# xdslproject/ExaHyPE

Hardware: AMD Instinct MI355X
Metric: DoF-updates/sec, 3D Euler p=5 fused STP+volume+Riemann, 1/2/4/8 MI355X (higher is better)
Workload: dtype f64

## Files before the change

### exahype_amd/csrc/exa_dg_reg.hpp

```cpp
#pragma once
#include "exa_dg_kernels.hpp"

namespace exa {

template <class P, class = void> struct pde_has_dir : std::false_type {};
template <class P> struct pde_has_dir<P, std::void_t<typename P::Dir>> : std::true_type {};

template <class PDE, bool HAS = pde_has_dir<PDE>::value> struct DirFlux;
template <class PDE> struct DirFlux<PDE, true> {
    typename PDE::Dir c;
    __device__ inline DirFlux(int d, double sc) { PDE::dir_init(c, d, sc); }
    __device__ inline void operator()(const double* q, const double* a, double* F) const { PDE::flux_scaled_dir(q, a, c, F); }
    __device__ inline double scale() const {
        double a = c.psc[0];
        asm volatile("" : "+v"(a));
        return (a + c.psc[1]) + c.psc[2];
    }
    __device__ inline void put(const double* pv, double vn, double sc, double* F) const { PDE::flux_scaled_put(pv, vn, c, sc, F); }
};
template <class PDE> struct DirFlux<PDE, false> {
    int d;
    double sc;
    __device__ inline DirFlux(int d_, double sc_) : d(d_), sc(sc_) {}
    __device__ inline void operator()(const double* q, const double* a, double* F) const {
        if (d == 0) PDE::template flux_scaled<0>(q, a, sc, F);
        else if (d == 1) PDE::template flux_scaled<1>(q, a, sc, F);
        else PDE::template flux_scaled<2>(q, a, sc, F);
    }
};

template <class P, class = void> struct pde_has_put : std::false_type {};
template <class P> struct pde_has_put<P, std::void_t<decltype(P::NPUT), decltype(P::PUT_VN)>> : std::true_type {};
template <class P, bool HAS = pde_has_put<P>::value> struct pde_nput { static constexpr int value = 0, vn = 0; };
template <class P> struct pde_nput<P, true> { static constexpr int value = P::NPUT, vn = P::PUT_VN; };

#ifndef EXA_REG_CPW
#define EXA_REG_CPW 2
#endif

template <int N> struct RegGeo {
    static constexpr int NN = N * N * N, NF = N * N;
    static constexpr int PY = N, PX = N * N;
    static constexpr int SL = NN + (NN % 2 == 0 ? 1 : 0);
    __host__ __device__ static constexpr int pstride(int d) { return d == 0 ? PX : (d == 1 ? PY : 1); }
    __host__ __device__ static inline int pbase(int d, int t) {
        const int a = t / N, b = t - a * N;
        return d == 0 ? a * PY + b : (d == 1 ? a * PX + b : a * PX + b * PY);
    }
};

template <int N, class PDE, int CPW = 1> struct StageAReg {
    using G = RegGeo<N>;
    static constexpr int NV = PDE::NV, NA = PDE::NAUX;
    static constexpr int NT = 256;
    static constexpr int LG = 2;
    static constexpr int LS = (N + LG - 1) / LG;
    static constexpr int VS = LG * G::SL;
    static constexpr int QSZ = NV * VS;
    static constexpr int NVA = NV + NA;
    static constexpr bool NCPV = pde_has_ncp<PDE>::value;
    static constexpr bool PUT = pde_has_put<PDE>::value && pde_has_dir<PDE>::value && !NCPV && !pde_has_xt<PDE>::value;
    static constexpr int NIMG = PUT ? pde_nput<PDE>::value : NVA;
    static constexpr int SOFF = NIMG * VS;
    static constexpr int GOFF = SOFF;
    static constexpr int PIC_D = SOFF + 3 * QSZ;
    static constexpr int FS = G::NN;
    static constexpr int FIN_D = (pde_has_source<PDE>::value ? 5 : 4) * NV * FS;
    static constexpr int CELL_D = PIC_D > FIN_D ? PIC_D : FIN_D;
    static constexpr size_t LDS_BYTES = sizeof(double) * ((size_t)CELL_D * CPW + 2 * 3 * N);
    static constexpr bool FITS = G::NN <= NT && 2 * sizeof(double) * (size_t)CELL_D + 2048 <= 160 * 1024;
    static constexpr int TAB_INTS = 2 * NT;
};

__device__ inline void lds_barrier() { __syncthreads(); }


template <int N, class PDE, int CPW, bool FUSE = false>
__global__ void __launch_bounds__(256 * CPW, 2)
dg_stage_a_reg_kernel(const double* u_in, double* u_out, double* __restrict__ trace,
                      long ncells, CellBox box, double dt, double idx0, double idx1, double idx2, int n_it,
                      const void* __restrict__ ops_raw, const int* __restrict__ tab, const void* __restrict__ step_raw, RegFuse fz, PlainGeo geo) {
    constexpr bool XT = pde_has_xt<PDE>::value, NCP = pde_has_ncp<PDE>::value;
    constexpr bool FXT = pde_flux_xt<PDE>::value;
    static_assert(!(FUSE && (XT || NCP)), "the one-kernel step is built for term sets without coordinates / ncp");
    using G = RegGeo<N>;
    using SA = StageAReg<N, PDE, CPW>;
    constexpr int NV = SA::NV, NA = SA::NA, DIM = 3;
    constexpr int NN = G::NN, NF = G::NF, SL = G::SL, PX = G::PX, PY = G::PY;
    constexpr int NT = SA::NT, LS = SA::LS, VS = SA::VS, QSZ = SA::QSZ, SOFF = SA::SOFF, FS = SA::FS, NVA = SA::NVA;
    [[maybe_unused]] constexpr int GOFF = SA::GOFF;
    constexpr bool PUT = SA::PUT;
    constexpr int NIMG = SA::NIMG, NLD = PUT ? NIMG + 1 : NVA;
    constexpr int H = N / 2;
    extern __shared__ __attribute__((aligned(16))) double lds_all[];
    const int half = __builtin_amdgcn_readfirstlane(threadIdx.x >> 8);
    const int tid = threadIdx.x & 255;
    __attribute__((address_space(3))) double* lds = (__attribute__((address_space(3))) double*)lds_all + half * SA::CELL_D;
    [[maybe_unused]] const int bt = (tid & 63) + 64 * half, grp = tid >> 6;
    EXA_STAMP_INIT();
    auto bar = [&]() {
        if constexpr (FUSE) {
            __builtin_amdgcn_fence(__ATOMIC_RELEASE, "workgroup", "local");
            __builtin_amdgcn_s_barrier();
            __builtin_amdgcn_fence(__ATOMIC_ACQUIRE, "workgroup", "local");
        } else {
            lds_barrier();
        }
    };
    const bool node_lane = tid < NN;
    const int o_n = node_lane ? tid : 0;
    const int pk2 = tab[tid], pk1 = tab[NT + tid];

    auto ld_group = [&](int base, int idx, auto& out) {
        constexpr int K = sizeof(out) / sizeof(double);
#pragma unroll
        for (int k = 0; k < K; k++) out[k] = EXA_LD(base + k * VS + idx);
    };
    auto st_group = [&](int base, int idx, const auto& in) {
        constexpr int K = sizeof(in) / sizeof(double);
#pragma unroll
        for (int k = 0; k < K; k++) EXA_ST(base + k * VS + idx, in[k]);
    };

    constexpr int NE = H * N + H + 1;
    struct Task {
        int off, ps, so;
        int vo;
        bool on;
        int d, ls;
        double xa, xb;
    };
    auto decode = [&](int pk, Task& k, DirFlux<PDE>& fx) {
        const int d = pk & 3, ls = (pk >> 2) & 1, t = pk >> 3;
        const int a = t / N, b = t - a * N;
        k.on = pk >= 0;
        k.off = ls * SL + (d == 0 ? a * PY + b : (d == 1 ? a * PX + b : a * PX + b * PY));
        k.ps = d == 0 ? PX : (d == 1 ? PY : 1);
        k.so = SOFF + d * QSZ;
        k.vo = PUT ? (pde_nput<PDE>::vn + d) * VS * (int)sizeof(double) : 0;
        k.d = d;
        k.ls = ls;
        if constexpr (XT) {
            k.xa = xi_of<N>(geo, a);
            k.xb = xi_of<N>(geo, b);
        }
        fx = DirFlux<PDE>(d, d == 0 ? idx0 : (d == 1 ? idx1 : idx2));
    };
    [[maybe_unused]] double xc[3] = {0.0, 0.0, 0.0};
    [[maybe_unused]] auto pencil_x = [&](const Task& tk, int d, int jn, double (&x)[3]) {
        const double xj = geo.xi[jn];
        x[0] = xc[0] + (d == 0 ? xj : tk.xa) * geo.h[0];
        x[1] = xc[1] + (d == 1 ? xj : (d == 0 ? tk.xa : tk.xb)) * geo.h[1];
        x[2] = xc[2] + (d == 2 ? xj : tk.xb) * geo.h[2];
    };
    [[maybe_unused]] double xio[3] = {0.0, 0.0, 0.0};
    if constexpr (XT) {
        xio[0] = xi_of<N>(geo, o_n / (N * N));
        xio[1] = xi_of<N>(geo, (o_n / N) % N);
        xio[2] = xi_of<N>(geo, o_n % N);
    }
    [[maybe_unused]] auto owner_x = [&](double (&x)[3]) {
#pragma unroll
        for (int a = 0; a < 3; a++) x[a] = xc[a] + xio[a] * geo.h[a];
    };
    [[maybe_unused]] auto level_t = [&](int l) -> double { return geo.t + geo.xi[l] * dt; };
    [[maybe_unused]] auto source_at = [&](const double* qv, int l, double* S) {
        if constexpr (pde_has_source<PDE>::value) {
            if constexpr (XT) {
                double x[3];
                owner_x(x);
                PDE::source_xt(qv, x, level_t(l), S);
            } else {
                PDE::source(qv, S);
            }
        }
    };
    Task tk2;
    DirFlux<PDE> fx2(0, 0.0);
    decode(pk2, tk2, fx2);
    bool active_now = true;
    static_assert(N % 2 == 0, "register-resident stage A: even N (the middle node of an odd N is not coded)");
    auto derive_a = [&](auto dc, const Task& tk, const DirFlux<PDE>& fx, double (&e)[H][NV], double (&o)[H][NV], [[maybe_unused]] double tA,
                        [[maybe_unused]] double tB) {
        constexpr int DC = decltype(dc)::value;
        if (tk.on && active_now) {
            const int off = tk.off, ps = tk.ps;
            double qa[N][NLD];
            auto ld_node = [&](int jn) {
                if constexpr (PUT) {
                    const volatile __attribute__((address_space(3))) double* a = &lds[off + jn * ps];
#pragma unroll
                    for (int k = 0; k < NIMG; k++) qa[jn][k] = a[k * VS];
                    const volatile __attribute__((address_space(3))) double* b;
                    asm volatile("v_add_u32 %0, %1, %2" : "=v"(b) : "v"(a), "v"(tk.vo));
                    qa[jn][NIMG] = *b;
                } else {
                    ld_group(0, off + jn * ps, qa[jn]);
                }
            };
#pragma unroll
            for (int j = 0; j < H; j++) {
                ld_node(j);
                ld_node(N - 1 - j);
            }
            [[maybe_unused]] double scl = 0.0;
            if constexpr (PUT) scl = fx.scale();
            [[maybe_unused]] const double tl = tk.ls ? tB : tA;
            [[maybe_unused]] const int dd = DC >= 0 ? DC : tk.d;
            [[maybe_unused]] const double scd = dd == 0 ? idx0 : (dd == 1 ? idx1 : idx2);
#pragma unroll
            for (int j = 0; j < H; j++) {
                double Fa[NV], Fb[NV];
                if constexpr (FXT) {
                    double xj[3];
                    pencil_x(tk, dd, j, xj);
                    dg_flux_xt<PDE>(qa[j], xj, tl, dd, Fa);
                    pencil_x(tk, dd, N - 1 - j, xj);
                    dg_flux_xt<PDE>(qa[N - 1 - j], xj, tl, dd, Fb);
#pragma unroll
                    for (int v = 0; v < NV; v++) { Fa[v] *= scd; Fb[v] *= scd; }
                } else if constexpr (DC >= 0) {
                    PDE::template flux_scaled<DC>(qa[j], qa[j] + NV, scd, Fa);
                    PDE::template flux_scaled<DC>(qa[N - 1 - j], qa[N - 1 - j] + NV, scd, Fb);
                } else if constexpr (PUT) {
                    fx.put(qa[j], qa[j][NIMG], scl, Fa);
                    fx.put(qa[N - 1 - j], qa[N - 1 - j][NIMG], scl, Fb);
                } else {
                    fx(qa[j], qa[j] + NV, Fa);
                    fx(qa[N - 1 - j], qa[N - 1 - j] + NV, Fb);
                }
#pragma unroll
                for (int v = 0; v < NV; v++) {
                    e[j][v] = Fa[v] + Fb[v];
                    o[j][v] = Fa[v] - Fb[v];
                }
            }
        }
    };
    [[maybe_unused]] auto derive_g = [&](const Task& tk, [[maybe_unused]] const double (&Em)[NE]) {
        if constexpr (NCP) {
            if (tk.on && active_now) {
                const int off = tk.off, ps = tk.ps, go = GOFF + tk.d * QSZ;
                const double scd = tk.d == 0 ? idx0 : (tk.d == 1 ? idx1 : idx2);
                double e[H][NV], o[H][NV];
#pragma unroll
                for (int j = 0; j < H; j++) {
                    double qa[NV], qb[NV];
                    ld_group(0, off + j * ps, qa);
                    ld_group(0, off + (N - 1 - j) * ps, qb);
#pragma unroll
                    for (int v = 0; v < NV; v++) {
                        e[j][v] = scd * (qa[v] + qb[v]);
                        o[j][v] = scd * (qa[v] - qb[v]);
                    }
                }
#pragma unroll
                for (int i = 0; i < H; i++) {
                    double M[NV], gI[NV], gM[NV];
#pragma unroll
                    for (int v = 0; v < NV; v++) M[v] = Em[H + i] * o[0][v];
#pragma unroll
                    for (int j = 1; j < H; j++)
#pragma unroll
                        for (int v = 0; v < NV; v++) EXA_FMA(M[v], Em[j * N + H + i], o[j][v]);
#pragma unroll
                    for (int v = 0; v < NV; v++) gI[v] = M[v];
#pragma unroll
                    for (int j = 0; j < H; j++)
#pragma unroll
                        for (int v = 0; v < NV; v++) EXA_FMA(gI[v], Em[j * N + i], e[j][v]);
#pragma unroll
                    for (int v = 0; v < NV; v++) gM[v] = fma(2.0, M[v], -gI[v]);
                    st_group(go, off + i * ps, gI);
                    st_group(go, off + (N - 1 - i) * ps, gM);
                }
            }
        }
    };
    [[maybe_unused]] auto ncp_at_owner = [&](const double* qv, int ls, int l, double (&out)[NV]) {
#pragma unroll
        for (int v = 0; v < NV; v++) out[v] = 0.0;
        if constexpr (NCP) {
            double xo[3] = {0.0, 0.0, 0.0};
            if constexpr (XT) owner_x(xo);
            static_for<0, DIM>([&](auto dc) {
                constexpr int D = decltype(dc)::value;
                double g[NV], nd[NV];
                ld_group(GOFF + D * QSZ, o_n + ls * SL, g);
#pragma unroll
                for (int v = 0; v < NV; v++) nd[v] = 0.0;
                dg_ncp<PDE>(qv, g, xo, XT ? level_t(l) : 0.0, D, nd);
#pragma unroll
                for (int v = 0; v < NV; v++) out[v] += nd[v];
            });
        }
    };
    auto derive_b = [&](const Task& tk, const double (&Em)[NE], const double (&e)[H][NV], const double (&o)[H][NV]) {
        if (tk.on && active_now) {
            const int off = tk.off, ps = tk.ps, so = PUT ? opaque_v(tk.so) : tk.so;
#pragma unroll
            for (int i = 0; i < H; i++) {
                double M[NV], sI[NV];
#pragma unroll
                for (int v = 0; v < NV; v++) M[v] = Em[H + i] * o[0][v];
#pragma unroll
                for (int j = 1; j < H; j++)
#pragma unroll
                    for (int v = 0; v < NV; v++) EXA_FMA(M[v], Em[j * N + H + i], o[j][v]);
#pragma unroll
                for (int v = 0; v < NV; v++) sI[v] = M[v];
#pragma unroll
                for (int j = 0; j < H; j++)
#pragma unroll
                    for (int v = 0; v < NV; v++) EXA_FMA(sI[v], Em[j * N + i], e[j][v]);
                double sM[NV];
#pragma unroll
                for (int v = 0; v < NV; v++) sM[v] = fma(2.0, M[v], -sI[v]);
                st_group(so, off + i * ps, sI);
                st_group(so, off + (N - 1 - i) * ps, sM);
            }
        }
    };
    using M0 = std::integral_constant<int, 0>;
    using M1 = std::integral_constant<int, 1>;
    using M2 = std::integral_constant<int, 2>;
    constexpr bool SPLIT_DIR = FXT || !pde_has_dir<PDE>::value;
    auto derive = [&](const Task& tk, const DirFlux<PDE>& fx, const double (&Em)[NE], double tA, double tB, auto mode) {
        __builtin_amdgcn_s_setprio(1);
        double e[H][NV], o[H][NV];
        constexpr int MODE = decltype(mode)::value;
        static_assert(!(NCP && MODE == 0), "gradients and sums share their arrays: two phases (M1, owners, M2)");
        if constexpr (MODE != 2) derive_g(tk, Em);
        auto front = [&](auto dc) {
            if constexpr (MODE != 1) derive_a(dc, tk, fx, e, o, tA, tB);
        };
        if constexpr (SPLIT_DIR) {
            if (tk.d == 0) front(std::integral_constant<int, 0>{});
            else if (tk.d == 1) front(std::integral_constant<int, 1>{});
            else front(std::integral_constant<int, 2>{});
        } else {
            front(std::integral_constant<int, -1>{});
        }
        if constexpr (MODE != 1) {
            derive_b(tk, Em, e, o);
        }
        __builtin_amdgcn_s_setprio(0);
    };

    int cx, cy, cz, sx, sy, sz;
    long trips;
    {
        const long b0 = (long)blockIdx.x * CPW + half, g = (long)gridDim.x * CPW;
        cz = (int)(b0 % box.nb[2]);
        cy = (int)((b0 / box.nb[2]) % box.nb[1]);
        cx = (int)(b0 / (box.nb[2] * box.nb[1]));
        sz = (int)(g % box.nb[2]);
        sy = (int)((g / box.nb[2]) % box.nb[1]);
        sx = (int)(g / (box.nb[2] * box.nb[1]));
        const long first = (long)blockIdx.x * CPW;
        trips = first < box.nbox ? (box.nbox - first + g - 1) / g : 0;
    }
    const int nb0 = (int)box.nb[0], nb1 = (int)box.nb[1], nb2 = (int)box.nb[2];
    auto cell_of = [&](int x, int y, int z) { return ((box.lo[0] + x) * box.nc[1] + box.lo[1] + y) * box.nc[2] + box.lo[2] + z; };
    double un[NV];
#pragma unroll
    for (int v = 0; v < NV; v++) un[v] = (node_lane && cx < nb0) ? u_in[(cell_of(cx, cy, cz) * NN + o_n) * NV + v] : 1.0;
    constexpr int TS = 2 * NV * NF;
    [[maybe_unused]] double tq[FUSE ? 4 : 1][NV];
    [[maybe_unused]] auto face_blocks = [&](int x, int y, int z, const double*& pm, const double*& pp, int& fyl) -> bool {
        const int lt = opaque_v(tid);
        const int f = lt / NF;
        fyl = lt - f * NF;
        const int d = f >> 1, side = f & 1;
        const int c0 = (int)box.lo[0] + x, c1 = (int)box.lo[1] + y, c2 = (int)box.lo[2] + z;
        const int n0 = (int)box.nc[0], n1 = (int)box.nc[1], n2 = (int)box.nc[2];
        const int cell = (c0 * n1 + c1) * n2 + c2;
        const int cst = d == 0 ? n1 * n2 : (d == 1 ? n2 : 1);
        const int ccd = d == 0 ? c0 : (d == 1 ? c1 : c2), ncd = d == 0 ? n0 : (d == 1 ? n1 : n2);
        const int tcell = d == 0 ? c1 * n2 + c2 : (d == 1 ? c0 * n2 + c2 : c0 * n1 + c1);
        const double* gh = f == 0 ? fz.ghost[0] : (f == 1 ? fz.ghost[1] : (f == 2 ? fz.ghost[2] : (f == 3 ? fz.ghost[3] : (f == 4 ? fz.ghost[4] : fz.ghost[5]))));
        const bool inner = side == 0 ? ccd > 0 : ccd < ncd - 1;
        const int nb = inner ? (side == 0 ? cell - cst : cell + cst) : (side == 0 ? cell + (ncd - 1) * cst : cell - (ncd - 1) * cst);
        const double* own = fz.trace_in + ((long)(d * 2 + side) * ncells + cell) * TS;
        const double* oth = (!inner && gh) ? gh + (long)tcell * TS : fz.trace_in + ((long)(d * 2 + 1 - side) * ncells + nb) * TS;
        pm = side == 0 ? oth : own;
        pp = side == 0 ? own : oth;
        return lt < 2 * DIM * NF && x < nb0;
    };
    [[maybe_unused]] auto fetch_faces = [&](int x, int y, int z) {
        if constexpr (FUSE) {
            const double *pm, *pp;
            int fyl;
#ifdef EXA_FUSE_ABL_NOLOAD
            const bool on = face_blocks(x, y, z, pm, pp, fyl) && false;
#else
            const bool on = face_blocks(x, y, z, pm, pp, fyl);
#endif
#pragma unroll
            for (int v = 0; v < NV; v++) {
                tq[0][v] = on ? pm[v * NF + fyl] : 1.0;
                tq[1][v] = on ? pp[v * NF + fyl] : 1.0;
                tq[2][v] = on ? pm[(NV + v) * NF + fyl] : 0.0;
                tq[3][v] = on ? pp[(NV + v) * NF + fyl] : 0.0;
            }
        }
    };
    constexpr int CWT = SA::CELL_D * CPW;
    if constexpr (FUSE) {
        if (threadIdx.x < 2 * DIM * N) {
            const DgOps<N>* og = reinterpret_cast<const DgOps<N>*>(ops_raw);
            const int t = threadIdx.x, D = t / (2 * N), sd = (t / N) & 1, i = t % N;
            const double idd = D == 0 ? idx0 : (D == 1 ? idx1 : idx2);
            ((__attribute__((address_space(3))) double*)lds_all)[CWT + t] = fz.dt_prev * idd * og->iw[i] * (sd == 0 ? og->phiL[i] : og->phiR[i]);
        }
    }
    fetch_faces(cx, cy, cz);
    if constexpr (CPW == 2) {
        if (half == 1) bar();
    }

    constexpr bool DEFER = FUSE;
    [[maybe_unused]] double upend[NV];
    [[maybe_unused]] long pend_cell = -1;
#pragma unroll
    for (int v = 0; v < NV; v++) upend[v] = 0.0;
    for (long trip = 0; trip < trips; trip++) {
        const bool active = cx < nb0;
        active_now = active;
        const bool owner = node_lane && active;
        const long cell = active ? cell_of(cx, cy, cz) : 0;
        if constexpr (XT) {
            xc[0] = geo.x0[0] + (double)(box.lo[0] + cx) * geo.h[0];
            xc[1] = geo.x0[1] + (double)(box.lo[1] + cy) * geo.h[1];
            xc[2] = geo.x0[2] + (double)(box.lo[2] + cz) * geo.h[2];
        }
        cz += sz;
        if (cz >= nb2) { cz -= nb2; cy += 1; }
        cy += sy;
        if (cy >= nb1) { cy -= nb1; cx += 1; }
        cx += sx;

        double q[N][NV];
        double Em[NE];
        sload<NE>(ops_here<N>(ops_raw)->DEO, Em);

        auto put_level = [&](int ls, const double (&qv)[NV]) {
            if constexpr (PUT) {
                double pv[NIMG];
                PDE::put_fast(qv, pv);
                st_group(0, o_n + ls * SL, pv);
            } else {
                double qa[NVA];
#pragma unroll
                for (int v = 0; v < NV; v++) qa[v] = qv[v];
                PDE::aux_fast(qv, qa + NV);
                st_group(0, o_n + ls * SL, qa);
            }
        };
#ifdef EXA_FUSE_ABL_NOPROLOGUE
        if constexpr (FUSE) {
            if (tq[0][0] == 1.2345e-300) un[0] += tq[1][1] + tq[2][2] + tq[3][3];
        }
        if constexpr (false) {
#else
        if constexpr (FUSE) {
#endif
            constexpr int LAM = SOFF, FSO = SOFF + NT;
            const int lt = opaque_v(tid);
            const int ff = lt / NF, fy = lt - ff * NF;
            const bool face_lane = lt < 2 * DIM * NF;
            const int d = ff >> 1;
            const double lam = face_lane ? fmax(PDE::maxeig_fast(tq[0], d), PDE::maxeig_fast(tq[1], d)) : 0.0;
            EXA_ST(LAM + tid, lam);
            bar();
            if (face_lane) {
                double lv[NF];
#pragma unroll
                for (int y = 0; y < NF; y++) lv[y] = EXA_LD(LAM + ff * NF + y);
#pragma unroll
                for (int st = 1; st < NF; st *= 2)
#pragma unroll
                    for (int y = 0; y + st < NF; y += 2 * st) lv[y] = fmax(lv[y], lv[y + st]);
                const double sm = lv[0];
#pragma unroll
                for (int v = 0; v < NV; v++) EXA_ST(FSO + (ff * NV + v) * NF + fy, 0.5 * (tq[2][v] + tq[3][v]) - 0.5 * sm * (tq[1][v] - tq[0][v]));
            }
            bar();
            if (owner) {
                static_for<0, DIM>([&](auto dc) {
                    constexpr int D = decltype(dc)::value;
                    const int on_ = opaque_v(o_n);
                    const int i = (on_ / G::pstride(D)) % N;
                    const int yy = D == 0 ? on_ % (N * N) : (D == 1 ? (on_ / (N * N)) * N + on_ % N : on_ / N);
                    const __attribute__((address_space(3))) double* cwt = (const __attribute__((address_space(3))) double*)lds_all + CWT + D * 2 * N;
                    const double cwL = cwt[i], cwR = cwt[N + i];
#pragma unroll
                    for (int v = 0; v < NV; v++) {
                        const double fL = EXA_LD(FSO + ((2 * D + 0) * NV + v) * NF + yy), fR = EXA_LD(FSO + ((2 * D + 1) * NV + v) * NF + yy);
                        un[v] -= cwR * fR - cwL * fL;
                    }
                });
                if (fz.u_plain) {
#pragma unroll
                    for (int v = 0; v < NV; v++) fz.u_plain[(cell * NN + o_n) * NV + v] = un[v];
                }
            }
        }
        double ukeep[NV];
#pragma unroll
        for (int v = 0; v < NV; v++) ukeep[v] = un[v];
        if constexpr (DEFER) {
            if (node_lane && pend_cell >= 0) {
                double* uo = u_out + (pend_cell * NN + o_n) * NV;
#pragma unroll
                for (int v = 0; v < NV; v++) uo[v] = upend[v];
            }
        }
        if constexpr (XT) {
#pragma unroll
            for (int l = 0; l < N; l++)
#pragma unroll
                for (int v = 0; v < NV; v++) q[l][v] = owner ? un[v] : 1.0;
        } else {
            if (owner) put_level(0, un);
            EXA_STAMP(0);
            bar();
            EXA_STAMP(1);
            [[maybe_unused]] double nd0[NV];
            {
                Task tk1;
                DirFlux<PDE> fx1(0, 0.0);
                decode(opaque_v(pk1), tk1, fx1);
                if constexpr (NCP) {
                    derive(tk1, fx1, Em, 0.0, 0.0, M1{});
                    bar();
                    if (owner) ncp_at_owner(un, 0, 0, nd0);
                    bar();
                    derive(tk1, fx1, Em, 0.0, 0.0, M2{});
                } else {
                    derive(tk1, fx1, Em, 0.0, 0.0, M0{});
                }
            }
            EXA_STAMP(2);
            bar();
            EXA_STAMP(3);
            if (owner) {
                double S[NV], Ts[N];
                sload<N>(step_here<N>(step_raw)->Tsdt, Ts);
                {
                    double Sx[NV], Sy[NV], Sz[NV];
                    ld_group(SOFF, o_n, Sx);
                    ld_group(SOFF + QSZ, o_n, Sy);
                    ld_group(SOFF + 2 * QSZ, o_n, Sz);
    #pragma unroll
                    for (int v = 0; v < NV; v++) S[v] = Sx[v] + (Sy[v] + Sz[v]);
                }
                if constexpr (pde_has_source<PDE>::value) {
                    double Sq[NV];
                    PDE::source(un, Sq);
    #pragma unroll
                    for (int v = 0; v < NV; v++) S[v] -= Sq[v];
                }
                if constexpr (NCP) {
    #pragma unroll
                    for (int v = 0; v < NV; v++) S[v] += nd0[v];
                }
    #pragma unroll
                for (int l = 0; l < N; l++)
    #pragma unroll
                    for (int v = 0; v < NV; v++) q[l][v] = fma(Ts[l], S[v], un[v]);
            } else {
    #pragma unroll
                for (int l = 0; l < N; l++)
    #pragma unroll
                    for (int v = 0; v < NV; v++) q[l][v] = 1.0;
            }
            EXA_STAMP(4);

        }
        auto load_levels = [&](auto lc, const double (&qq)[N][NV]) {
            constexpr int l0 = decltype(lc)::value;
            constexpr int NL = (l0 + 1 < N) ? 2 : 1;
#pragma unroll
            for (int ls = 0; ls < NL; ls++) put_level(ls, qq[l0 + ls]);
        };
        constexpr int IT0 = XT ? 0 : 1;
        if constexpr (PUT) decode(opaque_v(pk2), tk2, fx2);
        if (n_it > IT0 && owner) load_levels(std::integral_constant<int, 0>{}, q);
        constexpr bool DEFER_FOLD = NCP || XT;
        for (int it = IT0; it < n_it; it++) {
            double acc[N][NV];
            [[maybe_unused]] double Sk[DEFER_FOLD ? N : 1][NV];
            static_for<0, LS>([&](auto sc_) {
                constexpr int st = decltype(sc_)::value;
                constexpr int l0 = st * 2;
                constexpr int NL = (l0 + 1 < N) ? 2 : 1;
                sload<NE>(ops_here<N>(ops_raw)->DEO, Em);
                EXA_STAMP(5);
                bar();
                EXA_STAMP(6);
                static_assert(NL == 2, "odd N: the last step of an iteration has one level -- mask the tasks of level slot 1");
                [[maybe_unused]] double ndk[NL][NV];
                if constexpr (NCP) {
                    derive(tk2, fx2, Em, XT ? level_t(l0) : 0.0, XT ? level_t(l0 + 1) : 0.0, M1{});
                    bar();
                    if (owner) {
#pragma unroll
                        for (int ls = 0; ls < NL; ls++) ncp_at_owner(q[l0 + ls], ls, l0 + ls, ndk[ls]);
                    }
                    bar();
                    derive(tk2, fx2, Em, XT ? level_t(l0) : 0.0, XT ? level_t(l0 + 1) : 0.0, M2{});
                } else {
                    derive(tk2, fx2, Em, XT ? level_t(l0) : 0.0, XT ? level_t(l0 + 1) : 0.0, M0{});
                }
                [[maybe_unused]] double Tm[NL * N], uu[NV];
                if constexpr (!DEFER_FOLD) {
#pragma unroll
                    for (int k = 0; k < NL * N; k++) Tm[k] = step_here<N>(step_raw)->TdtT[l0 * N + k];
                    if constexpr (st == 0) {
#pragma unroll
                        for (int v = 0; v < NV; v++) uu[v] = ukeep[v];
                    }
                }
                EXA_STAMP(7);
                bar();
                EXA_STAMP(8);
                if (owner) {
                    if constexpr (!DEFER_FOLD) spin(Tm);
                    double Sx[NL][NV], Sy[NL][NV], Sz[NL][NV];
#pragma unroll
                    for (int ls = 0; ls < NL; ls++) {
                        ld_group(SOFF, o_n + ls * SL, Sx[ls]);
                        ld_group(SOFF + QSZ, o_n + ls * SL, Sy[ls]);
                        ld_group(SOFF + 2 * QSZ, o_n + ls * SL, Sz[ls]);
                    }
                    if constexpr (st + 1 < LS) load_levels(std::integral_constant<int, l0 + 2>{}, q);
                    __builtin_amdgcn_sched_barrier(0);
#pragma unroll
                    for (int ls = 0; ls < NL; ls++)
#pragma unroll
                        for (int v = 0; v < NV; v++) Sx[ls][v] += Sy[ls][v] + Sz[ls][v];
                    if constexpr (pde_has_source<PDE>::value) {
#pragma unroll
                        for (int ls = 0; ls < NL; ls++) {
                            double Sq[NV];
                            source_at(q[l0 + ls], l0 + ls, Sq);
#pragma unroll
                            for (int v = 0; v < NV; v++) Sx[ls][v] -= Sq[v];
                        }
                    }
                    if constexpr (NCP) {
#pragma unroll
                        for (int ls = 0; ls < NL; ls++)
#pragma unroll
                            for (int v = 0; v < NV; v++) Sx[ls][v] += ndk[ls][v];
                    }
                    if constexpr (DEFER_FOLD) {
#pragma unroll
                        for (int ls = 0; ls < NL; ls++)
#pragma unroll
                            for (int v = 0; v < NV; v++) Sk[l0 + ls][v] = Sx[ls][v];
                        if constexpr (st + 1 == LS) {
                            static_for<0, LS>([&](auto s2_) {
                                constexpr int s2 = decltype(s2_)::value;
                                constexpr int m0 = s2 * 2;
                                double T2[NL * N];
                                sload<NL * N>(step_here<N>(step_raw)->TdtT + m0 * N, T2);
#pragma unroll
                                for (int ls = 0; ls < NL; ls++)
#pragma unroll
                                    for (int lp = 0; lp < N; lp++)
#pragma unroll
                                        for (int v = 0; v < NV; v++)
                                            acc[lp][v] = fma(T2[ls * N + lp], Sk[m0 + ls][v], (s2 == 0 && ls == 0) ? ukeep[v] : acc[lp][v]);
                            });
                        }
                    } else {
#pragma unroll
                    for (int ls = 0; ls < NL; ls++)
#pragma unroll
                        for (int lp = 0; lp < N; lp++)
#pragma unroll
                            for (int v = 0; v < NV; v++) {
                                if constexpr (st == 0) acc[lp][v] = fma(Tm[ls * N + lp], Sx[ls][v], ls == 0 ? uu[v] : acc[lp][v]);
                                else acc[lp][v] = fma(Tm[ls * N + lp], Sx[ls][v], acc[lp][v]);
                            }
                    }
                    if constexpr (st + 1 == LS) {
                        if (it + 1 < n_it) load_levels(std::integral_constant<int, 0>{}, acc);
                    }
                }
                EXA_STAMP(9);
            });
#pragma unroll
            for (int l = 0; l < N; l++)
#pragma unroll
                for (int v = 0; v < NV; v++) q[l][v] = owner ? acc[l][v] : 1.0;
        }

        [[maybe_unused]] double pw[NV];
        if constexpr (NCP) {
#pragma unroll
            for (int v = 0; v < NV; v++) pw[v] = 0.0;
            if (owner) load_levels(std::integral_constant<int, 0>{}, q);
            static_for<0, LS>([&](auto sc_) {
                constexpr int st = decltype(sc_)::value;
                constexpr int l0 = st * 2;
                sload<NE>(ops_here<N>(ops_raw)->DEO, Em);
                bar();
                derive(tk2, fx2, Em, XT ? level_t(l0) : 0.0, XT ? level_t(l0 + 1) : 0.0, M1{});
                bar();
                if (owner) {
                    double wl[2];
                    sload<2>(ops_here<N>(ops_raw)->w + l0, wl);
#pragma unroll
                    for (int ls = 0; ls < 2; ls++) {
                        double nd[NV];
                        ncp_at_owner(q[l0 + ls], ls, l0 + ls, nd);
#pragma unroll
                        for (int v = 0; v < NV; v++) pw[v] = fma(wl[ls], nd[v], pw[v]);
                    }
                    if constexpr (st + 1 < LS) load_levels(std::integral_constant<int, l0 + 2>{}, q);
                }
            });
        }
        bar();
        if (owner) {
            double wm[N];
            sload<N>(ops_here<N>(ops_raw)->w, wm);
            double qb[NV], Fb[DIM][NV];
            [[maybe_unused]] double Sbar[NV];
#pragma unroll
            for (int v = 0; v < NV; v++) qb[v] = 0.0;
#pragma unroll
            for (int d = 0; d < DIM; d++)
#pragma unroll
                for (int v = 0; v < NV; v++) Fb[d][v] = 0.0;
            if constexpr (pde_has_source<PDE>::value) {
#pragma unroll
                for (int v = 0; v < NV; v++) Sbar[v] = 0.0;
            }
#pragma unroll
            for (int l = 0; l < N; l++) {
                double a[nz(NA)], F[NV];
                PDE::aux_fast(q[l], a);
#pragma unroll
                for (int v = 0; v < NV; v++) qb[v] += wm[l] * q[l][v];
                static_for<0, DIM>([&](auto dc) {
                    constexpr int D = decltype(dc)::value;
                    if constexpr (FXT) {
                        double xo[3];
                        owner_x(xo);
                        dg_flux_xt<PDE>(q[l], xo, level_t(l), D, F);
                    } else {
                        PDE::template flux<D>(q[l], a, F);
                    }
#pragma unroll
                    for (int v = 0; v < NV; v++) Fb[D][v] += wm[l] * F[v];
                });
                if constexpr (pde_has_source<PDE>::value) {
                    double Sq[NV];
                    source_at(q[l], l, Sq);
#pragma unroll
                    for (int v = 0; v < NV; v++) Sbar[v] += wm[l] * Sq[v];
                }
            }
#pragma unroll
            for (int v = 0; v < NV; v++) {
                EXA_ST(v * FS + o_n, qb[v]);
#pragma unroll
                for (int d = 0; d < DIM; d++) EXA_ST(((1 + d) * NV + v) * FS + o_n, Fb[d][v]);
                if constexpr (pde_has_source<PDE>::value) EXA_ST((4 * NV + v) * FS + o_n, Sbar[v]);
            }
        }
        EXA_STAMP(10);
        bar();

#pragma unroll
        for (int v = 0; v < NV; v++) un[v] = (node_lane && cx < nb0) ? u_in[(cell_of(cx, cy, cz) * NN + o_n) * NV + v] : 1.0;
        fetch_faces(cx, cy, cz);

        {
            double KE[NE], iwm[N], pl[N], pr[N];
            sload<NE>(ops_here<N>(ops_raw)->KEO, KE);
            sload<N>(ops_here<N>(ops_raw)->iw, iwm);
            sload<N>(ops_here<N>(ops_raw)->phiL, pl);
            sload<N>(ops_here<N>(ops_raw)->phiR, pr);
            static_assert(NV * NF <= NT, "closing phases: one round per direction");
            const int tv = PUT ? opaque_v(tid) : tid;
            const int v = tv / NF, t = tv - v * NF;
            static_for<0, DIM>([&](auto dc) {
                constexpr int D = decltype(dc)::value;
                if (tid < NV * NF) {
                    constexpr int ps = G::pstride(D);
                    const int pb = G::pbase(D, t);
                    double qb[N], Fb[N], vol[N];
#pragma unroll
                    for (int j = 0; j < N; j++) {
                        qb[j] = EXA_LD(v * FS + pb + j * ps);
                        Fb[j] = EXA_LD(((1 + D) * NV + v) * FS + pb + j * ps);
                    }
                    eo_apply<N>(KE, Fb, vol);
                    const double sc = dt * (D == 0 ? idx0 : (D == 1 ? idx1 : idx2));
#pragma unroll
                    for (int i = 0; i < N; i++) EXA_ST(((1 + D) * NV + v) * FS + pb + i * ps, sc * iwm[i] * vol[i]);
                    double qL = 0.0, qR = 0.0, FL = 0.0, FR = 0.0;
#pragma unroll
                    for (int j = 0; j < N; j++) {
                        qL += pl[j] * qb[j];
                        qR += pr[j] * qb[j];
                        FL += pl[j] * Fb[j];
                        FR += pr[j] * Fb[j];
                    }
                    if (active) {
                        double* tl = trace + (((long)D * 2 + 0) * ncells + cell) * (2 * NV * NF);
                        double* tr = trace + (((long)D * 2 + 1) * ncells + cell) * (2 * NV * NF);
                        tl[(0 * NV + v) * NF + t] = qL;
                        tl[(1 * NV + v) * NF + t] = FL;
                        tr[(0 * NV + v) * NF + t] = qR;
                        tr[(1 * NV + v) * NF + t] = FR;
                    }
                }
            });
        }
        EXA_STAMP(11);
        bar();

        if (owner) {
            double us[NV];
#pragma unroll
            for (int v2 = 0; v2 < NV; v2++) {
                us[v2] = ukeep[v2];
                if constexpr (NCP) us[v2] -= dt * pw[v2];
                if constexpr (pde_has_source<PDE>::value) us[v2] += dt * EXA_LD((4 * NV + v2) * FS + o_n);
#pragma unroll
                for (int d = 0; d < DIM; d++) us[v2] += EXA_LD(((1 + d) * NV + v2) * FS + o_n);
            }
            if constexpr (DEFER) {
#pragma unroll
                for (int v2 = 0; v2 < NV; v2++) upend[v2] = us[v2];
            } else {
                double* uo = u_out + (cell * NN + o_n) * NV;
#pragma unroll
                for (int v2 = 0; v2 < NV; v2++) uo[v2] = us[v2];
            }
        }
        if constexpr (DEFER) pend_cell = active ? cell : -1;
        bar();
    }
    if constexpr (DEFER) {
        if (node_lane && pend_cell >= 0) {
            double* uo = u_out + (pend_cell * NN + o_n) * NV;
#pragma unroll
            for (int v = 0; v < NV; v++) uo[v] = upend[v];
        }
    }
    if constexpr (CPW == 2) {
        if (half == 0) bar();
    }
    EXA_STAMP_FLUSH();
}

}
```

Baseline: 13.58 billion.

## Relocate closing LDS image past aux area to drop end-of-trip barrier

Moves the closing-phase LDS arrays (q, fluxes, source) to start after the aux image region (offset SOFF) and pads them to the SL stride, so the closing data no longer overlaps what the next trip's prologue writes. This lets the kernel skip the end-of-trip barrier when not fused and not coordinate-dependent. It also makes the stagger between the two cells sharing a workgroup configurable as an odd number of barrier phases. The change relies on the closing image fitting inside the prologue footprint (asserted) and on the removed barrier really being unnecessary; any hidden read/write overlap would be a race.

```diff
diff --git a/exahype_amd/csrc/exa_dg_reg.hpp b/exahype_amd/csrc/exa_dg_reg.hpp
--- a/exahype_amd/csrc/exa_dg_reg.hpp
+++ b/exahype_amd/csrc/exa_dg_reg.hpp
@@ -37,6 +37,10 @@
 #ifndef EXA_REG_CPW
 #define EXA_REG_CPW 2
 #endif
+#ifndef EXA_REG_OFFSET
+#define EXA_REG_OFFSET 1
+#endif
+static_assert(EXA_REG_OFFSET > 0 && EXA_REG_OFFSET % 2 == 1, "EXA_REG_OFFSET: odd, or the two cells in flight derive at the same time");
 
 template <int N> struct RegGeo {
     static constexpr int NN = N * N * N, NF = N * N;
@@ -64,9 +68,10 @@
     static constexpr int SOFF = NIMG * VS;
     static constexpr int GOFF = SOFF;
     static constexpr int PIC_D = SOFF + 3 * QSZ;
-    static constexpr int FS = G::NN;
-    static constexpr int FIN_D = (pde_has_source<PDE>::value ? 5 : 4) * NV * FS;
-    static constexpr int CELL_D = PIC_D > FIN_D ? PIC_D : FIN_D;
+    static constexpr int FS = G::SL;
+    static constexpr int FIN_D = SOFF + (pde_has_source<PDE>::value ? 5 : 4) * NV * FS;
+    static_assert(FIN_D <= PIC_D && G::NN <= G::SL, "the closing image lies inside the arrays of the sums");
+    static constexpr int CELL_D = PIC_D;
     static constexpr size_t LDS_BYTES = sizeof(double) * ((size_t)CELL_D * CPW + 2 * 3 * N);
     static constexpr bool FITS = G::NN <= NT && 2 * sizeof(double) * (size_t)CELL_D + 2048 <= 160 * 1024;
     static constexpr int TAB_INTS = 2 * NT;
@@ -89,6 +94,7 @@
     constexpr int NN = G::NN, NF = G::NF, SL = G::SL, PX = G::PX, PY = G::PY;
     constexpr int NT = SA::NT, LS = SA::LS, VS = SA::VS, QSZ = SA::QSZ, SOFF = SA::SOFF, FS = SA::FS, NVA = SA::NVA;
     [[maybe_unused]] constexpr int GOFF = SA::GOFF;
+    constexpr int CB = SOFF;
     constexpr bool PUT = SA::PUT;
     constexpr int NIMG = SA::NIMG, NLD = PUT ? NIMG + 1 : NVA;
     constexpr int H = N / 2;
@@ -416,7 +422,10 @@
     }
     fetch_faces(cx, cy, cz);
     if constexpr (CPW == 2) {
-        if (half == 1) bar();
+        if (half == 1) {
+#pragma unroll 1
+            for (int k = 0; k < EXA_REG_OFFSET; k++) bar();
+        }
     }
 
     constexpr bool DEFER = FUSE;
@@ -767,10 +776,10 @@
             }
 #pragma unroll
             for (int v = 0; v < NV; v++) {
-                EXA_ST(v * FS + o_n, qb[v]);
-#pragma unroll
-                for (int d = 0; d < DIM; d++) EXA_ST(((1 + d) * NV + v) * FS + o_n, Fb[d][v]);
-                if constexpr (pde_has_source<PDE>::value) EXA_ST((4 * NV + v) * FS + o_n, Sbar[v]);
+                EXA_ST(CB + v * FS + o_n, qb[v]);
+#pragma unroll
+                for (int d = 0; d < DIM; d++) EXA_ST(CB + ((1 + d) * NV + v) * FS + o_n, Fb[d][v]);
+                if constexpr (pde_has_source<PDE>::value) EXA_ST(CB + (4 * NV + v) * FS + o_n, Sbar[v]);
             }
         }
         EXA_STAMP(10);
@@ -797,13 +806,13 @@
                     double qb[N], Fb[N], vol[N];
 #pragma unroll
                     for (int j = 0; j < N; j++) {
-                        qb[j] = EXA_LD(v * FS + pb + j * ps);
-                        Fb[j] = EXA_LD(((1 + D) * NV + v) * FS + pb + j * ps);
+                        qb[j] = EXA_LD(CB + v * FS + pb + j * ps);
+                        Fb[j] = EXA_LD(CB + ((1 + D) * NV + v) * FS + pb + j * ps);
                     }
                     eo_apply<N>(KE, Fb, vol);
                     const double sc = dt * (D == 0 ? idx0 : (D == 1 ? idx1 : idx2));
 #pragma unroll
-                    for (int i = 0; i < N; i++) EXA_ST(((1 + D) * NV + v) * FS + pb + i * ps, sc * iwm[i] * vol[i]);
+                    for (int i = 0; i < N; i++) EXA_ST(CB + ((1 + D) * NV + v) * FS + pb + i * ps, sc * iwm[i] * vol[i]);
                     double qL = 0.0, qR = 0.0, FL = 0.0, FR = 0.0;
 #pragma unroll
                     for (int j = 0; j < N; j++) {
@@ -832,9 +841,9 @@
             for (int v2 = 0; v2 < NV; v2++) {
                 us[v2] = ukeep[v2];
                 if constexpr (NCP) us[v2] -= dt * pw[v2];
-                if constexpr (pde_has_source<PDE>::value) us[v2] += dt * EXA_LD((4 * NV + v2) * FS + o_n);
-#pragma unroll
-                for (int d = 0; d < DIM; d++) us[v2] += EXA_LD(((1 + d) * NV + v2) * FS + o_n);
+                if constexpr (pde_has_source<PDE>::value) us[v2] += dt * EXA_LD(CB + (4 * NV + v2) * FS + o_n);
+#pragma unroll
+                for (int d = 0; d < DIM; d++) us[v2] += EXA_LD(CB + ((1 + d) * NV + v2) * FS + o_n);
             }
             if constexpr (DEFER) {
 #pragma unroll
@@ -846,7 +855,8 @@
             }
         }
         if constexpr (DEFER) pend_cell = active ? cell : -1;
-        bar();
+        constexpr bool END_BAR = FUSE || XT;
+        if constexpr (END_BAR) bar();
     }
     if constexpr (DEFER) {
         if (node_lane && pend_cell >= 0) {
@@ -856,7 +866,10 @@
         }
     }
     if constexpr (CPW == 2) {
-        if (half == 0) bar();
+        if (half == 0) {
+#pragma unroll 1
+            for (int k = 0; k < EXA_REG_OFFSET; k++) bar();
+        }
     }
     EXA_STAMP_FLUSH();
 }
```

Measured after the change: 13.77 billion (median of 6 runs). 1.01x the previous value.
